# DCASE-REPO/DESED_task

Hardware: AMD Instinct MI355X
Metric: 10s-clips/sec CRNN mean-teacher train @batch48 (higher is better)
Workload: dtype f32 (fp32 storage and accumulation; the dense contractions of the wide layers run as split-bf16 MFMA, 3 bf16 products per fp32 product, fp32-level accuracy; everything else exact f32)

## Files before the change

desed_task_amd/_lib.py:

```python
import ctypes
import os
import re

_HERE = os.path.dirname(os.path.abspath(__file__))
_HEADER = os.path.join(os.path.dirname(_HERE), "include", "sed_hip.h")
LIB_PATH = os.path.join(_HERE, "libsed_hip.so")

_CTYPES = {"int": ctypes.c_int, "float": ctypes.c_float, "double": ctypes.c_double, "long long": ctypes.c_longlong,
           "unsigned": ctypes.c_uint, "unsigned int": ctypes.c_uint}

ERRORS = {-1: "bad argument", -2: "kernel launch failed", -3: "unsupported configuration"}


def parse_header(path=_HEADER):
    text = open(path).read()
    text = re.sub(r"/\*.*?\*/", "", text, flags=re.S)
    protos = {}
    for m in re.finditer(r"\b(?:int|long long)\s+(sed_\w+)\s*\(([^)]*)\)\s*;", text):
        args = []
        for a in m.group(2).split(","):
            a = a.strip()
            if "*" in a:
                args.append(ctypes.c_void_p)
            else:
                ty = re.sub(r"\bconst\b", "", a).strip()
                ty = ty.rsplit(None, 1)[0].strip()
                args.append(_CTYPES[ty])
        protos[m.group(1)] = args
    return protos


def header_constants(path=_HEADER):
    return {m.group(1): int(m.group(2)) for m in re.finditer(r"^#define\s+(SED_\w+)\s+(\d+)\b", open(path).read(), re.M)}


class _Lib:
    def __init__(self, path, is_emulator=False):
        self.path = path
        self.is_emulator = is_emulator
        import torch
        self._dll = ctypes.CDLL(path)
        self.protos = parse_header()
        for name, argtypes in self.protos.items():
            fn = getattr(self._dll, name)
            fn.argtypes = argtypes
            fn.restype = ctypes.c_longlong if name.endswith("_floats") else ctypes.c_int

    def value(self, name, *args):
        return getattr(self._dll, name)(*args)

    def call(self, name, *args):
        rc = getattr(self._dll, name)(*args)
        if rc != 0:
            raise RuntimeError("%s failed: %s (rc=%d)" % (name, ERRORS.get(rc, "?"), rc))


_lib = None


def get():
    global _lib
    if _lib is None:
        if not os.path.exists(LIB_PATH):
            raise RuntimeError(
                "desed_task_amd: %s is missing -- build it with `python -m desed_task_amd.build` "
                "(hipcc --offload-arch=gfx950).  There is no CPU fallback." % LIB_PATH)
        _lib = _Lib(LIB_PATH)
    return _lib


def use_library(path, is_emulator=True):
    global _lib
    _lib = _Lib(path, is_emulator=is_emulator) if path is not None else None
    return _lib


TUNING_KEYS = {"glu_grid_cap": 0, "glu_bwd128_split": 1, "convb_ck": 2, "convb_mp": 3, "block0_nocenter": 4, "glu_fwd128": 5, "wgrad_narrow": 6, "wgrad_cap": 7, "attn_valu": 8, "wgrad_wide": 9, "gru_lds_kb": 10, "mel_taps_mem": 11, "convb_tpw": 12, "mel_wave": 13, "gemm_ntn": 14, "linear_tiles": 15}


_tuning = {}


def set_tuning(key, value):
    get().call("sed_set_tuning", TUNING_KEYS[key], int(value))
    _tuning[key] = int(value)


def get_tuning(key):
    return _tuning.get(key, 0)


def check_tensor(t, name="tensor"):
    lib = get()
    if lib.is_emulator:
        if t.is_cuda:
            raise RuntimeError("%s: emulator build bound but tensor is on the GPU" % name)
    elif not t.is_cuda:
        raise RuntimeError("%s must live on the MI355X (cuda) device: there is no CPU path" % name)
    if not t.is_contiguous():
        raise RuntimeError("%s must be contiguous" % name)


def stream_ptr(t):
    if t.is_cuda:
        import torch
        return torch.cuda.current_stream(t.device).cuda_stream
    return 0
```

desed_task_amd/csrc/sed_common.h:

```cpp
#pragma once

#ifdef SED_EMU
#include "hip_emu.h"
#else
#include <hip/hip_runtime.h>
#define SED_DYN_SMEM(name) extern __shared__ __attribute__((aligned(16))) char name[]
#define SED_LAUNCH(kern, grid, block, smem, stream, ...) \
    hipLaunchKernelGGL(kern, grid, block, smem, stream, __VA_ARGS__)
typedef float f32x16 __attribute__((ext_vector_type(16)));
typedef float f32x4 __attribute__((ext_vector_type(4)));
typedef short s16x8 __attribute__((ext_vector_type(8)));
#endif

#include <stdint.h>

#define SED_API extern "C" __attribute__((visibility("default")))

#define SED_MAX_SMEM(kern, bytes) \
    (void)hipFuncSetAttribute((const void*)(kern), hipFuncAttributeMaxDynamicSharedMemorySize, (int)(bytes))

__global__ __launch_bounds__(256) static void sed_zero4_kernel(float* p0, int n0, float* p1, int n1, float* p2, int n2, float* p3, int n3) {
    const int i = blockIdx.x * 256 + threadIdx.x;
    if (i < n0) p0[i] = 0.f;
    if (i < n1) p1[i] = 0.f;
    if (i < n2) p2[i] = 0.f;
    if (i < n3) p3[i] = 0.f;
}
static inline void sed_zero4(hipStream_t s, float* p0, int n0, float* p1, int n1, float* p2, int n2, float* p3, int n3) {
    int n = n0 > n1 ? n0 : n1;
    n = n > n2 ? n : n2;
    n = n > n3 ? n : n3;
    if (n <= 0) return;
    SED_LAUNCH(sed_zero4_kernel, dim3((n + 255) / 256), dim3(256), 0, s, p0, n0, p1, n1, p2, n2, p3, n3);
}

#define SED_OK 0
#define SED_ERR_ARG (-1)
#define SED_ERR_LAUNCH (-2)
#define SED_ERR_UNSUPPORTED (-3)

enum { SED_TUNE_GLU_GRID_CAP = 0, SED_TUNE_GLU_BWD128_SPLIT = 1, SED_TUNE_CONVB_CK = 2, SED_TUNE_CONVB_MP = 3, SED_TUNE_B0_NOCENTER = 4, SED_TUNE_GLU_FWD128 = 5, SED_TUNE_WGRAD_NARROW = 6, SED_TUNE_WGRAD_CAP = 7,
       SED_TUNE_ATTN_VALU = 8, SED_TUNE_WGRAD_WIDE = 9, SED_TUNE_GRU_LDS_KB = 10, SED_TUNE_MEL_TAPS_MEM = 11, SED_TUNE_CONVB_TPW = 12, SED_TUNE_MEL_WAVE = 13, SED_TUNE_GEMM_NTN = 14, SED_TUNE_LINEAR_TILES = 15, SED_TUNE_COUNT = 16 };
extern int sed_tuning[SED_TUNE_COUNT];

static inline int sed_check_launch() {
    hipError_t e = hipGetLastError();
    return e == hipSuccess ? SED_OK : SED_ERR_LAUNCH;
}

__device__ __forceinline__ f32x16 mfma32(float a, float b, f32x16 c) {
#ifdef SED_EMU
    return emu_mfma_32x32x2(a, b, c);
#else
    return __builtin_amdgcn_mfma_f32_32x32x2f32(a, b, c, 0, 0, 0);
#endif
}
__device__ __forceinline__ int mfma32_row(int r, int lane) { return (r & 3) + 8 * (r >> 2) + 4 * (lane >> 5); }

__device__ __forceinline__ f32x4 mfma16(float a, float b, f32x4 c) {
#ifdef SED_EMU
    return emu_mfma_16x16x4(a, b, c);
#else
    return __builtin_amdgcn_mfma_f32_16x16x4f32(a, b, c, 0, 0, 0);
#endif
}

__device__ __forceinline__ f32x16 mfma32_bf16(s16x8 a, s16x8 b, f32x16 c) {
#ifdef SED_EMU
    return emu_mfma_32x32x16_bf16(a, b, c);
#else
    typedef __bf16 bf16x8_t __attribute__((ext_vector_type(8)));
    return __builtin_amdgcn_mfma_f32_32x32x16_bf16(__builtin_bit_cast(bf16x8_t, a), __builtin_bit_cast(bf16x8_t, b), c, 0, 0, 0);
#endif
}
__device__ __forceinline__ f32x4 mfma16_bf16(s16x8 a, s16x8 b, f32x4 c) {
#ifdef SED_EMU
    return emu_mfma_16x16x32_bf16(a, b, c);
#else
    typedef __bf16 bf16x8_t __attribute__((ext_vector_type(8)));
    return __builtin_amdgcn_mfma_f32_16x16x32_bf16(__builtin_bit_cast(bf16x8_t, a), __builtin_bit_cast(bf16x8_t, b), c, 0, 0, 0);
#endif
}
__device__ __forceinline__ unsigned short f32_to_bf16(float x) {
    unsigned u = __float_as_uint(x);
    u += 0x7FFFu + ((u >> 16) & 1u);
    return (unsigned short)(u >> 16);
}
__device__ __forceinline__ float bf16_to_f32(unsigned short h) { return __uint_as_float(((unsigned)h) << 16); }
__device__ __forceinline__ void bf16_split(float x, unsigned short& hi, unsigned short& lo) {
    hi = f32_to_bf16(x);
    lo = f32_to_bf16(x - bf16_to_f32(hi));
}

__device__ __forceinline__ float sed_sadd(float a, float b) {
#ifdef SED_EMU
    return a + b;
#else
    float r;
    asm("v_add_f32 %0, %1, %2" : "=v"(r) : "v"(a), "v"(b));
    return r;
#endif
}

__device__ __forceinline__ float sed_sfma(float a, float b, float c) {
#ifdef SED_EMU
    return fmaf(a, b, c);
#else
    float r;
    asm("v_fma_f32 %0, %1, %2, %3" : "=v"(r) : "v"(a), "v"(b), "v"(c));
    return r;
#endif
}

__device__ __forceinline__ void sed_sched_fence() {
#ifndef SED_EMU
    __builtin_amdgcn_sched_barrier(0);
#endif
}

__device__ __forceinline__ unsigned sed_alignbit(unsigned hi, unsigned lo, unsigned shift) {
#ifdef SED_EMU
    return (unsigned)(((((unsigned long long)hi) << 32) | lo) >> shift);
#else
    return __builtin_amdgcn_alignbit(hi, lo, shift);
#endif
}

template <class T_>
__device__ __forceinline__ void sed_pin(T_& x) {
#ifndef SED_EMU
    asm volatile("" : "+v"(x));
#else
    (void)x;
#endif
}
__device__ __forceinline__ void sed_opaque(int& x) {
#ifndef SED_EMU
    asm volatile("" : "+v"(x));
#else
    (void)x;
#endif
}

__device__ __forceinline__ int sed_wave_uniform(int x) {
#ifdef SED_EMU
    return x;
#else
    return __builtin_amdgcn_readfirstlane(x);
#endif
}

__device__ __forceinline__ void sed_wave_sync() {
#ifdef SED_EMU
    emu_wave_sync();
#else
    __builtin_amdgcn_fence(__ATOMIC_ACQ_REL, "wavefront");
    __builtin_amdgcn_wave_barrier();
#endif
}

__device__ __forceinline__ void bf16_split2(float a, float b, unsigned& hi, unsigned& lo) {
#ifdef SED_EMU
    unsigned short h0, l0, h1, l1;
    bf16_split(a, h0, l0);
    bf16_split(b, h1, l1);
    hi = (unsigned)h0 | ((unsigned)h1 << 16);
    lo = (unsigned)l0 | ((unsigned)l1 << 16);
#else
    typedef float f32x2_t __attribute__((ext_vector_type(2)));
    typedef __bf16 bf16x2_t __attribute__((ext_vector_type(2)));
    const f32x2_t v = {a, b};
    hi = __builtin_bit_cast(unsigned, __builtin_convertvector(v, bf16x2_t));
    const f32x2_t hf = {__uint_as_float(hi << 16), __uint_as_float(hi & 0xFFFF0000u)};
    lo = __builtin_bit_cast(unsigned, __builtin_convertvector(v - hf, bf16x2_t));
#endif
}
struct SedOneProduct {};
template <class... ONE>
constexpr int sed_np() { return sizeof...(ONE) ? 1 : 3; }
__device__ __forceinline__ unsigned bf16_round2(float a, float b) {
#ifdef SED_EMU
    return (unsigned)f32_to_bf16(a) | ((unsigned)f32_to_bf16(b) << 16);
#else
    typedef float f32x2_t __attribute__((ext_vector_type(2)));
    typedef __bf16 bf16x2_t __attribute__((ext_vector_type(2)));
    const f32x2_t v = {a, b};
    return __builtin_bit_cast(unsigned, __builtin_convertvector(v, bf16x2_t));
#endif
}

__device__ __forceinline__ f32x16 f32x16_zero() {
    f32x16 z;
#pragma unroll
    for (int i = 0; i < 16; ++i) z[i] = 0.f;
    return z;
}

__device__ __forceinline__ float sed_quad_xor1(float v) {
#ifdef SED_EMU
    return __shfl_xor(v, 1);
#else
    return __builtin_bit_cast(float, __builtin_amdgcn_update_dpp(0, __builtin_bit_cast(int, v), 0xB1, 0xF, 0xF, true));
#endif
}
__device__ __forceinline__ float sed_quad_xor2(float v) {
#ifdef SED_EMU
    return __shfl_xor(v, 2);
#else
    return __builtin_bit_cast(float, __builtin_amdgcn_update_dpp(0, __builtin_bit_cast(int, v), 0x4E, 0xF, 0xF, true));
#endif
}
__device__ __forceinline__ float sed_row_ror4(float v) {
#ifdef SED_EMU
    return __shfl_xor(v, 4);
#else
    return __builtin_bit_cast(float, __builtin_amdgcn_update_dpp(0, __builtin_bit_cast(int, v), 0x124, 0xF, 0xF, true));
#endif
}
__device__ __forceinline__ float sed_row_ror8(float v) {
#ifdef SED_EMU
    return __shfl_xor(v, 8);
#else
    return __builtin_bit_cast(float, __builtin_amdgcn_update_dpp(0, __builtin_bit_cast(int, v), 0x128, 0xF, 0xF, true));
#endif
}
__device__ __forceinline__ float sed_row16_max(float v) {
    v = fmaxf(v, sed_quad_xor1(v)); v = fmaxf(v, sed_quad_xor2(v));
    v = fmaxf(v, sed_row_ror4(v)); v = fmaxf(v, sed_row_ror8(v));
    return v;
}
__device__ __forceinline__ float sed_row16_sum(float v) {
    v += sed_quad_xor1(v); v += sed_quad_xor2(v);
    v += sed_row_ror4(v); v += sed_row_ror8(v);
    return v;
}
__device__ __forceinline__ float sed_half_mirror(float v) {
#ifdef SED_EMU
    return __shfl_xor(v, 7);
#else
    return __builtin_bit_cast(float, __builtin_amdgcn_update_dpp(0, __builtin_bit_cast(int, v), 0x141, 0xF, 0xF, true));
#endif
}
__device__ __forceinline__ float sed_quad_sum(float v) {
    v += sed_quad_xor1(v);
    v += sed_quad_xor2(v);
    return v;
}

__device__ __forceinline__ float wave_sum(float v) {
#pragma unroll
    for (int m = 32; m >= 1; m >>= 1) v += __shfl_xor(v, m);
    return v;
}
__device__ __forceinline__ float wave_min(float v) {
#pragma unroll
    for (int m = 32; m >= 1; m >>= 1) v = fminf(v, __shfl_xor(v, m));
    return v;
}
__device__ __forceinline__ float wave_max(float v) {
#pragma unroll
    for (int m = 32; m >= 1; m >>= 1) v = fmaxf(v, __shfl_xor(v, m));
    return v;
}

__device__ __forceinline__ uint32_t sed_mix32(uint32_t x) {
    x ^= x >> 16; x *= 0x85EBCA6Bu;
    x ^= x >> 13; x *= 0xC2B2AE35u;
    x ^= x >> 16;
    return x;
}
__device__ __forceinline__ uint32_t sed_hash(uint32_t idx, uint32_t seed) {
// ... 153 lines not shown
```

desed_task_amd/csrc/sed_conv.hip:

```cpp
#include "sed_common.h"

__global__ __launch_bounds__(256) void pack_weights_kernel(const float* __restrict__ W, float* __restrict__ Wf,
                                                           float* __restrict__ Wd, int COUT, int CIN) {
    const int i = blockIdx.x * 256 + threadIdx.x;
    if (i >= COUT * CIN * 9) return;
    const int b = i % 3, a = (i / 3) % 3, ci = (i / 9) % CIN, co = i / (9 * CIN);
    const float w = W[i];
    Wf[((a * 3 + b) * CIN + ci) * COUT + co] = w;
    if (Wd) Wd[(((2 - a) * 3 + (2 - b)) * COUT + co) * CIN + ci] = w;
}
SED_API int sed_conv_pack_weights(const float* W, float* Wf, float* Wd, int COUT, int CIN, void* stream) {
    const int n = COUT * CIN * 9;
    SED_LAUNCH(pack_weights_kernel, dim3((n + 255) / 256), dim3(256), 0, (hipStream_t)stream, W, Wf, Wd, COUT, CIN);
    return sed_check_launch();
}
struct PackJobs {
    const float* W[8];
    float* Wf[8];
    float* Wd[8];
    int cout[8], cin[8], start[9];
    int n;
};
__global__ __launch_bounds__(256) void pack_weights_multi_kernel(PackJobs jobs) {
    const int i = blockIdx.x * 256 + threadIdx.x;
// ... 463 lines not shown
            constexpr int NX = KT * (CIN / 4) / 256, ND = KT * (COUT / 4) / 256;
            float4 lx[NX], ldy[ND];
#pragma unroll
            for (int u = 0; u < NX; ++u) {
                const int idx = tid + 256 * u, r = idx / (CIN / 4), v = idx - r * (CIN / 4);
                const int p = p0 + r;
                lx[u] = make_float4(0.f, 0.f, 0.f, 0.f);
                if (p < npix) {
                    const int f = p % F, t = (p / F) % T, bb = p / (F * T);
                    const int t2 = t + da, f2 = f + db;
                    if (t2 >= 0 && t2 < T && f2 >= 0 && f2 < F)
                        lx[u] = *(const float4*)(x + (((size_t)bb * T + t2) * F + f2) * CIN + 4 * v);
                }
            }
#pragma unroll
            for (int u = 0; u < ND; ++u) {
                const int idx = tid + 256 * u, r = idx / (COUT / 4), v = idx - r * (COUT / 4);
                const int p = p0 + r;
                ldy[u] = make_float4(0.f, 0.f, 0.f, 0.f);
                if (p < npix) ldy[u] = *(const float4*)(dy + (size_t)p * COUT + 4 * v);
            }
#pragma unroll
            for (int u = 0; u < NX; ++u) {
                const int idx = tid + 256 * u, r = idx / (CIN / 4), v = idx - r * (CIN / 4);
                *(float4*)(xs + r * CIN + 4 * v) = lx[u];
            }
#pragma unroll
            for (int u = 0; u < ND; ++u) {
                const int idx = tid + 256 * u, r = idx / (COUT / 4), v = idx - r * (COUT / 4);
                *(float4*)(ds + r * COUT + 4 * v) = ldy[u];
            }
        }
        __syncthreads();
        constexpr int KS = KT / WK;
#pragma unroll 4
        for (int k = wk * KS; k < (wk + 1) * KS; k += 2) {
            float av[MT];
#pragma unroll
            for (int m = 0; m < MT; ++m) av[m] = (CIN >= 32 || lo < CIN) ? xs[(k + hi) * CIN + m * 32 + lo] : 0.f;
#pragma unroll
            for (int n = 0; n < NTW; ++n) {
                const int co = (wn * NTW + n) * 32 + lo;
                const float bv = (COUT >= 32 || lo < COUT) ? ds[(k + hi) * COUT + co] : 0.f;
#pragma unroll
                for (int m = 0; m < MT; ++m) acc[m][n] = mfma32(av[m], bv, acc[m][n]);
            }
        }
    }
    static_assert(WK == 1, "wide layers: every wave owns its output tiles");
    float* part = dWp + ((size_t)blockIdx.x * 9 + tap) * CIN * COUT;
#pragma unroll
    for (int m = 0; m < MT; ++m)
#pragma unroll
        for (int n = 0; n < NTW; ++n) {
            const int co = (wn * NTW + n) * 32 + lo;
#pragma unroll
            for (int r = 0; r < 16; ++r) {
                const int ci = m * 32 + mfma32_row(r, lane);
                if (ci < CIN && co < COUT) part[(size_t)ci * COUT + co] = acc[m][n][r];
            }
        }
}

template <int CIN, int COUT>
static int launch_wgrad(const float* x, const float* dy, float* dWp, int B, int T, int F, hipStream_t s) {
    using Cfg = WgCfg<CIN, COUT>;
    const int splits = wgrad_parts(CIN, COUT, B, T, F);
    SED_MAX_SMEM((conv_wgrad_kernel<CIN, COUT>), Cfg::SMEM);
    SED_LAUNCH((conv_wgrad_kernel<CIN, COUT>), dim3(splits, 9), dim3(256), Cfg::SMEM, s, x, dy, dWp, B, T, F);
    return sed_check_launch();
}

template <int CIN, int COUT, int NP = 3>
struct WgbCfg {
    static constexpr int PLANES = NP == 1 ? 1 : 2;
    static constexpr int KT = 64, RS = 64;
    static constexpr int MT = CIN / 32, NT = COUT / 32;
    static constexpr int WM = MT >= 4 ? 2 : 1, WN = 4 / WM;
    static constexpr int MTW = MT / WM, NTW = NT / WN;
    static constexpr int NBX = (KT / 4) * (CIN / 4) / 256, NBD = (KT / 4) * (COUT / 4) / 256;
    static constexpr int SMEM = PLANES * (CIN + COUT) * RS * 2;
    static_assert(NBX >= 1 && NBD >= 1 && MTW * WM == MT && NTW * WN == NT, "tile split");
};

template <bool LO = true>
__device__ __forceinline__ void wgb_store_row(float a, float b, float c, float d, unsigned short* __restrict__ hi_row,
                                              unsigned short* __restrict__ lo_row) {
    if constexpr (!LO) {
        *(uint2*)hi_row = make_uint2(bf16_round2(a, b), bf16_round2(c, d));
    } else {
    uint2 h, l;
    bf16_split2(a, b, h.x, l.x);
    bf16_split2(c, d, h.y, l.y);
    *(uint2*)hi_row = h;
    *(uint2*)lo_row = l;
    }
}
template <bool LO = true>
__device__ __forceinline__ void wgb_store_block(const float4 v0, const float4 v1, const float4 v2, const float4 v3,
                                                unsigned short* __restrict__ hi_plane, unsigned short* __restrict__ lo_plane,
                                                int cq, int pq, int RS) {
    const int r0 = 4 * cq, f0 = (r0 ^ cq) & 7;
    const int o0 = r0 * RS + 4 * (pq ^ (2 * f0)), o1 = (r0 + 1) * RS + 4 * (pq ^ (2 * (f0 ^ 1)));
    const int o2 = (r0 + 2) * RS + 4 * (pq ^ (2 * (f0 ^ 2))), o3 = (r0 + 3) * RS + 4 * (pq ^ (2 * (f0 ^ 3)));
    wgb_store_row<LO>(v0.x, v1.x, v2.x, v3.x, hi_plane + o0, lo_plane + o0);
    wgb_store_row<LO>(v0.y, v1.y, v2.y, v3.y, hi_plane + o1, lo_plane + o1);
    wgb_store_row<LO>(v0.z, v1.z, v2.z, v3.z, hi_plane + o2, lo_plane + o2);
    wgb_store_row<LO>(v0.w, v1.w, v2.w, v3.w, hi_plane + o3, lo_plane + o3);
}

template <int CIN, int COUT, class... ONE>
__global__ __launch_bounds__(256) void conv_wgrad_bf16_kernel(const float* __restrict__ x, const float* __restrict__ dy,
                                                              float* __restrict__ dWp, int B, int T, int F) {
    constexpr int NP = sed_np<ONE...>();
    using Cfg = WgbCfg<CIN, COUT, NP>;
    constexpr int KT = Cfg::KT, RS = Cfg::RS, WN = Cfg::WN, MTW = Cfg::MTW, NTW = Cfg::NTW, NBX = Cfg::NBX, NBD = Cfg::NBD;
    SED_DYN_SMEM(smem);
    unsigned short* xh = (unsigned short*)smem;
    unsigned short* xl = xh + (Cfg::PLANES - 1) * CIN * RS;
    unsigned short* dh = xl + CIN * RS;
    unsigned short* dl = dh + (Cfg::PLANES - 1) * COUT * RS;
    const int tid = threadIdx.x, lane = tid & 63, w = tid >> 6, lo = lane & 31, hi = lane >> 5;
    const int wn = w % WN, wm = w / WN;
    const int tap = blockIdx.y, da = tap / 3 - 1, db = tap % 3 - 1;
    const int npix = B * T * F;
    const int ntiles = (npix + KT - 1) / KT;
    const int fsh = 31 - __builtin_clz(F);

    f32x16 acc[MTW][NTW];
#pragma unroll
    for (int m = 0; m < MTW; ++m)
#pragma unroll
        for (int n = 0; n < NTW; ++n) acc[m][n] = f32x16_zero();

    float4 rx[NBX * 4], rd[NBD * 4];
    unsigned okx = 0, okd = 0;
    static_assert(NBX * 4 <= 32 && NBD * 4 <= 32, "validity masks");
    auto load_tile = [&](int tile) {
        const int p0 = tile * KT;
        okx = 0; okd = 0;
#pragma unroll
        for (int u = 0; u < NBX; ++u) {
            const int blk = tid + 256 * u, cq = (blk >> 1) % (CIN / 4), pq = (blk & 1) + 2 * ((blk >> 1) / (CIN / 4));
#pragma unroll
            for (int j = 0; j < 4; ++j) {
                const int p = p0 + 4 * pq + j, pc = p < npix ? p : 0;
                const int f = pc & (F - 1), tt = pc >> fsh, t = tt % T, bb = tt / T;
                const int t2 = t + da, f2 = f + db;
                const bool ok = p < npix && t2 >= 0 && t2 < T && f2 >= 0 && f2 < F;
                okx |= (ok ? 1u : 0u) << (4 * u + j);
                const int t2c = t2 < 0 ? 0 : (t2 >= T ? T - 1 : t2), f2c = f2 < 0 ? 0 : (f2 >= F ? F - 1 : f2);
                rx[4 * u + j] = *(const float4*)(x + (((size_t)bb * T + t2c) * F + f2c) * CIN + 4 * cq);
            }
        }
#pragma unroll
        for (int u = 0; u < NBD; ++u) {
            const int blk = tid + 256 * u, cq = (blk >> 1) % (COUT / 4), pq = (blk & 1) + 2 * ((blk >> 1) / (COUT / 4));
#pragma unroll
            for (int j = 0; j < 4; ++j) {
                const int p = p0 + 4 * pq + j;
                okd |= (p < npix ? 1u : 0u) << (4 * u + j);
                rd[4 * u + j] = *(const float4*)(dy + (size_t)(p < npix ? p : 0) * COUT + 4 * cq);
            }
        }
    };
    auto store_tile = [&]() {
#pragma unroll
        for (int i = 0; i < NBX * 4; ++i) if (!((okx >> i) & 1u)) rx[i] = make_float4(0.f, 0.f, 0.f, 0.f);
#pragma unroll
        for (int i = 0; i < NBD * 4; ++i) if (!((okd >> i) & 1u)) rd[i] = make_float4(0.f, 0.f, 0.f, 0.f);
#pragma unroll
        for (int u = 0; u < NBX; ++u) {
            const int blk = tid + 256 * u;
            wgb_store_block<NP != 1>(rx[4 * u], rx[4 * u + 1], rx[4 * u + 2], rx[4 * u + 3], xh, xl, (blk >> 1) % (CIN / 4),
                            (blk & 1) + 2 * ((blk >> 1) / (CIN / 4)), RS);
        }
#pragma unroll
        for (int u = 0; u < NBD; ++u) {
            const int blk = tid + 256 * u;
            wgb_store_block<NP != 1>(rd[4 * u], rd[4 * u + 1], rd[4 * u + 2], rd[4 * u + 3], dh, dl, (blk >> 1) % (COUT / 4),
                            (blk & 1) + 2 * ((blk >> 1) / (COUT / 4)), RS);
        }
    };

    int tile = blockIdx.x;
    if (tile < ntiles) load_tile(tile);
    for (; tile < ntiles; tile += gridDim.x) {
        __syncthreads();
        store_tile();
        __syncthreads();
        if (tile + (int)gridDim.x < ntiles) load_tile(tile + gridDim.x);
#pragma unroll
// ... 784 lines not shown
```

desed_task_amd/csrc/sed_gemm_bf16.hip:

```cpp
#include "sed_common.h"

namespace {

constexpr int GB_BM = 128, GB_BK = 32, GB_RS = 40;

__device__ __forceinline__ void split4(const float4 v, uint2& h, uint2& l) {
    bf16_split2(v.x, v.y, h.x, l.x);
    bf16_split2(v.z, v.w, h.y, l.y);
}
__device__ __forceinline__ uint2 round4(const float4 v) { return make_uint2(bf16_round2(v.x, v.y), bf16_round2(v.z, v.w)); }

template <int ROWS, bool KC>
struct OperandTile {
    static constexpr int NV = ROWS * GB_BK / 4 / 256;
    float4 r[NV];
    static __device__ __forceinline__ int kc_row(int i) {
        const int grp = i >> 4;
        return ((grp >> 2) << 3) + (grp & 3) + ((i >> 1) & 4);
    }
    __device__ __forceinline__ void load(const float* __restrict__ base, int ld, int row0, int nrows, int k0, int kend, int tid) {
#pragma unroll
        for (int u = 0; u < NV; ++u) {
            r[u] = make_float4(0.f, 0.f, 0.f, 0.f);
            if (KC) {
// ... 48 lines not shown
    }
};

template <int TA, int TB, int NTN, class... ONE>
__global__ __launch_bounds__(256, 3) void gemm_bf16x3_kernel(const float* __restrict__ A, const float* __restrict__ Bm,
                                                          const float* __restrict__ bias, float* __restrict__ Cm, int M, int N, int K,
                                                          int lda, int ldb, int ldc, int k_per_slice, int atomic,
                                                          const float* __restrict__ A1, const float* __restrict__ B1,
                                                          const float* __restrict__ bias1, float* __restrict__ C1, int nbatch,
                                                          const float* __restrict__ Bsw, int ksw, int act, float* __restrict__ part,
                                                          int walk_nt) {
    constexpr int NP = sed_np<ONE...>();
    constexpr int BM = GB_BM, BN = 32 * NTN, BK = GB_BK, RS = GB_RS;
    constexpr int PLANES = NP == 1 ? 1 : 2;
    __shared__ __attribute__((aligned(16))) unsigned short As[PLANES * BM * RS];
    __shared__ __attribute__((aligned(16))) unsigned short Bs[PLANES * BN * RS];
    const int tid = threadIdx.x, lane = tid & 63, w = tid >> 6, lo = lane & 31, hi = lane >> 5;
    int tile_m = blockIdx.y, tile_n = blockIdx.x;
    if (walk_nt > 0) {
        const int ml = blockIdx.x >> 3;
        tile_m = (blockIdx.x & 7) + 8 * (ml / walk_nt);
        tile_n = ml % walk_nt;
        if (tile_m * BM >= M) return;
    }
    const int m0 = tile_m * BM, n0 = tile_n * BN;
    const int zb = nbatch == 2 ? (blockIdx.z & 1) : 0, zs = nbatch == 2 ? (blockIdx.z >> 1) : blockIdx.z;
    if (zb) { A = A1; Bm = B1; bias = bias1; Cm = C1; }
    if (part) { Cm = part + (size_t)blockIdx.z * M * N; ldc = N; }
    const int kbeg = zs * k_per_slice, kend = min(K, kbeg + k_per_slice);
    f32x16 acc[NTN];
#pragma unroll
    for (int i = 0; i < NTN; ++i) acc[i] = f32x16_zero();
    OperandTile<BM, TA == 0> ta;
    OperandTile<BN, TB == 1> tb;

    if (kbeg < kend) { ta.load(A, lda, m0, M, kbeg, kend, tid); tb.load((Bsw && kbeg >= ksw) ? Bsw : Bm, ldb, n0, N, kbeg, kend, tid); }
    for (int k0 = kbeg; k0 < kend; k0 += BK) {
        __syncthreads();
        ta.template store<NP != 1>(As, As + BM * RS, tid);
        tb.template store<NP != 1>(Bs, Bs + BN * RS, tid);
        __syncthreads();
        if (k0 + BK < kend) { ta.load(A, lda, m0, M, k0 + BK, kend, tid); tb.load((Bsw && k0 + BK >= ksw) ? Bsw : Bm, ldb, n0, N, k0 + BK, kend, tid); }
        const unsigned short* ap = As + (32 * w + lo) * RS + 8 * hi;
#pragma unroll
        for (int ks = 0; ks < BK / 16; ++ks) {
            const s16x8 a_hi = *(const s16x8*)(ap + 16 * ks);
            if constexpr (NP == 1) {
#pragma unroll
                for (int nt = 0; nt < NTN; ++nt)
                    acc[nt] = mfma32_bf16(a_hi, *(const s16x8*)(Bs + (nt * 32 + lo) * RS + 16 * ks + 8 * hi), acc[nt]);
            } else {
            const s16x8 a_lo = *(const s16x8*)(ap + BM * RS + 16 * ks);
#pragma unroll
            for (int nt = 0; nt < NTN; ++nt) {
                const unsigned short* bp = Bs + (nt * 32 + lo) * RS + 16 * ks + 8 * hi;
                const s16x8 b_hi = *(const s16x8*)bp;
                const s16x8 b_lo = *(const s16x8*)(bp + BN * RS);
                acc[nt] = mfma32_bf16(a_lo, b_hi, acc[nt]);
                acc[nt] = mfma32_bf16(a_hi, b_lo, acc[nt]);
                acc[nt] = mfma32_bf16(a_hi, b_hi, acc[nt]);
            }
            }
        }
    }
#pragma unroll
    for (int nt = 0; nt < NTN; ++nt) {
        const int gn = n0 + nt * 32 + lo;
        if (gn < N) {
            const float bv = (bias != nullptr && zs == 0) ? bias[gn] : 0.f;
#pragma unroll
            for (int r = 0; r < 16; ++r) {
                const int gm = m0 + 32 * w + mfma32_row(r, lane);
                if (gm < M) {
                    float* dst = Cm + (size_t)gm * ldc + gn;
                    float v = acc[nt][r] + bv;
                    if (act == 1) v = 0.5f * v * (1.0f + erff(v * 0.70710678118654752f));
                    if (atomic) atomicAdd(dst, v); else *dst = v;
                }
            }
        }
    }
}

}

SED_API int sed_gemm(const float* A, const float* Bm, const float* bias, float* Cm, int M, int N, int K, int lda, int ldb,
                        int ldc, int transA, int transB, int split_k, int accumulate, void* stream);
SED_API int sed_gemm_pair(const float* A0, const float* A1, const float* B0, const float* B1, const float* bias0,
                             const float* bias1, float* C0, float* C1, int M, int N, int K, int lda, int ldb, int ldc, int transA,
                             int transB, int split_k, int accumulate, void* stream);

static int gemmb_dispatch(const float* A, const float* Bm, const float* bias, float* Cm, const float* A1, const float* B1,
                          const float* bias1, float* C1, int nbatch, int M, int N, int K, int lda, int ldb, int ldc, int transA,
                          int transB, int split_k, int accumulate, hipStream_t s, const float* Bsw = nullptr, int ksw = 0, int act = 0,
                          float* part = nullptr, bool act_linear = false, bool single = false) {
    if (M <= 0 || N <= 0 || K <= 0) return SED_OK;
    bool ok = ((uintptr_t)A % 16 == 0) && ((uintptr_t)Bm % 16 == 0) && lda % 4 == 0 && ldb % 4 == 0 &&
              ((transA ? M : K) % 4 == 0) && ((transB ? K : N) % 4 == 0) && !(transA && transB);
    if (nbatch == 2) ok = ok && ((uintptr_t)A1 % 16 == 0) && ((uintptr_t)B1 % 16 == 0);
    if (!ok && (Bsw || act || part)) return SED_ERR_UNSUPPORTED;
    if (!ok) {
        if (nbatch == 2) return sed_gemm_pair(A, A1, Bm, B1, bias, bias1, Cm, C1, M, N, K, lda, ldb, ldc, transA, transB, split_k, accumulate, s);
        return sed_gemm(A, Bm, bias, Cm, M, N, K, lda, ldb, ldc, transA, transB, split_k, accumulate, s);
    }
    if (split_k < 1) split_k = 1;
    int kps = ((K + split_k - 1) / split_k + 31) / 32 * 32;
    split_k = (K + kps - 1) / kps;
    const int atomic = (!part && (split_k > 1 || accumulate)) ? 1 : 0;
    int ntn = N > 64 ? 4 : 2;
    if (ntn == 4 && ((N + 127) / 128) * ((M + 127) / 128) * split_k * nbatch < 400) ntn = 2;
    if (ntn == 4 && !transA && transB && N % 96 == 0) {
        const long long rows = (M + 127) / 128, z = (long long)split_k * nbatch, slots = 768;
        const long long t4 = rows * ((N + 127) / 128) * z, t3 = rows * (N / 96) * z;
        if (sed_tuning[SED_TUNE_GEMM_NTN] == 3) ntn = 3;
        else if (t4 > slots) {
            const double e4 = (double)t4 / (double)(((t4 + slots - 1) / slots) * slots), e3 = (double)t3 / (double)(((t3 + slots - 1) / slots) * slots);
            if (e3 > e4 + 0.1) ntn = 3;
        }
    }
    dim3 grid((N + 32 * ntn - 1) / (32 * ntn), (M + 127) / 128, split_k * nbatch);
    int walk_nt = 0;
    if (act_linear && split_k * nbatch == 1 && grid.y >= 16) {
        walk_nt = (int)grid.x;
        grid = dim3(grid.x * ((grid.y + 7) / 8) * 8, 1, 1);
    }
#define GEMMB_CASE(ta, tb, nn) \
    if (single && transA == ta && transB == tb && ntn == nn) { SED_LAUNCH((gemm_bf16x3_kernel<ta, tb, nn, SedOneProduct>), grid, dim3(256), 0, s, A, Bm, bias, Cm, M, N, K, lda, ldb, ldc, kps, atomic, A1, B1, bias1, C1, nbatch, Bsw, ksw, act, part, walk_nt); return sed_check_launch(); }
    GEMMB_CASE(0, 0, 2) GEMMB_CASE(0, 0, 4) GEMMB_CASE(0, 1, 2) GEMMB_CASE(0, 1, 3) GEMMB_CASE(0, 1, 4) GEMMB_CASE(1, 0, 2) GEMMB_CASE(1, 0, 4)
#undef GEMMB_CASE
#define GEMMB_CASE(ta, tb, nn) \
    if (transA == ta && transB == tb && ntn == nn) { SED_LAUNCH((gemm_bf16x3_kernel<ta, tb, nn>), grid, dim3(256), 0, s, A, Bm, bias, Cm, M, N, K, lda, ldb, ldc, kps, atomic, A1, B1, bias1, C1, nbatch, Bsw, ksw, act, part, walk_nt); return sed_check_launch(); }
    GEMMB_CASE(0, 0, 2) GEMMB_CASE(0, 0, 4) GEMMB_CASE(0, 1, 2) GEMMB_CASE(0, 1, 3) GEMMB_CASE(0, 1, 4) GEMMB_CASE(1, 0, 2) GEMMB_CASE(1, 0, 4)
#undef GEMMB_CASE
    return SED_ERR_UNSUPPORTED;
}

SED_API int sed_gemm_bf16x3(const float* A, const float* Bm, const float* bias, float* Cm, int M, int N, int K, int lda, int ldb,
                               int ldc, int transA, int transB, int split_k, int accumulate, void* stream) {
    return gemmb_dispatch(A, Bm, bias, Cm, nullptr, nullptr, nullptr, nullptr, 1, M, N, K, lda, ldb, ldc, transA, transB, split_k,
                          accumulate, (hipStream_t)stream);
}
SED_API int sed_gemm_pair_bf16x3(const float* A0, const float* A1, const float* B0, const float* B1, const float* bias0,
                                    const float* bias1, float* C0, float* C1, int M, int N, int K, int lda, int ldb, int ldc,
                                    int transA, int transB, int split_k, int accumulate, void* stream) {
    return gemmb_dispatch(A0, B0, bias0, C0, A1, B1, bias1, C1, 2, M, N, K, lda, ldb, ldc, transA, transB, split_k, accumulate,
                          (hipStream_t)stream);
}

__global__ __launch_bounds__(256) void splitk_reduce_kernel(const float* __restrict__ part, float* __restrict__ C0, float* __restrict__ C1,
                                                            int nslices, int M, int N, int ldc) {
    const int MN4 = M * N / 4, i = blockIdx.x * 256 + threadIdx.x, zb = blockIdx.y, nb = gridDim.y;
    if (i >= MN4) return;
    const float4* src = (const float4*)part + (size_t)zb * MN4 + i;
    float4 acc = make_float4(0.f, 0.f, 0.f, 0.f);
#pragma unroll 4
    for (int z = 0; z < nslices; ++z) {
        const float4 v = src[(size_t)nb * z * MN4];
        acc.x += v.x; acc.y += v.y; acc.z += v.z; acc.w += v.w;
    }
    const int e = 4 * i, m = e / N, n = e - m * N;
    *(float4*)((zb ? C1 : C0) + (size_t)m * ldc + n) = acc;
}
static inline int splitk_slices(int K, int split_k) {
    if (split_k < 1) split_k = 1;
    const int kps = ((K + split_k - 1) / split_k + 31) / 32 * 32;
    return (K + kps - 1) / kps;
}
SED_API long long sed_gemm_splitk_scratch_floats(int M, int N, int K, int split_k) {
    return 2LL * splitk_slices(K, split_k) * M * N;
}
SED_API int sed_gemm_pair_splitk_bf16x3(const float* A0, const float* A1, const float* B0, const float* B1, float* C0, float* C1,
                                           int M, int N, int K, int lda, int ldb, int ldc, int transA, int transB, int split_k,
                                           float* scratch, void* stream) {
    if (M <= 0 || N <= 0) return SED_OK;
    if (!scratch || N % 4 != 0 || ldc % 4 != 0 || K <= 0) return SED_ERR_ARG;
    if ((((uintptr_t)C0 | (uintptr_t)C1) & 15) != 0) return SED_ERR_UNSUPPORTED;
    hipStream_t s = (hipStream_t)stream;
    const int rc = gemmb_dispatch(A0, B0, nullptr, C0, A1, B1, nullptr, C1, 2, M, N, K, lda, ldb, ldc, transA, transB, split_k, 0, s,
                                  nullptr, 0, 0, scratch);
    if (rc != SED_OK) return rc;
    SED_LAUNCH(splitk_reduce_kernel, dim3((M * N / 4 + 255) / 256, 2), dim3(256), 0, s, (const float*)scratch, C0, C1,
               splitk_slices(K, split_k), M, N, ldc);
    return sed_check_launch();
}

SED_API int sed_gemm_splitk_bf16x3(const float* A, const float* Bm, float* Cm, int M, int N, int K, int lda, int ldb, int ldc,
                                   int transA, int transB, int split_k, float* scratch, void* stream) {
    if (M <= 0 || N <= 0) return SED_OK;
    if (!scratch || N % 4 != 0 || ldc % 4 != 0 || K <= 0) return SED_ERR_ARG;
    if (((uintptr_t)Cm & 15) != 0) return SED_ERR_UNSUPPORTED;
    hipStream_t s = (hipStream_t)stream;
// ... 728 lines not shown
```

desed_task_amd/csrc/sed_selftest.hip:

```cpp
#include "sed_common.h"

int sed_tuning[SED_TUNE_COUNT] = {0};
SED_API int sed_set_tuning(int key, int value) {
    if (key < 0 || key >= SED_TUNE_COUNT) return SED_ERR_ARG;
    sed_tuning[key] = value;
    return SED_OK;
}

__global__ __launch_bounds__(64) void selftest_mfma32_kernel(const float* A, const float* Bm, float* C, int K) {
    const int lane = threadIdx.x;
    f32x16 acc = f32x16_zero();
    for (int k = 0; k < K; k += 2) {
        const float a = A[(lane & 31) * K + k + (lane >> 5)];
        const float b = Bm[(k + (lane >> 5)) * 32 + (lane & 31)];
        acc = mfma32(a, b, acc);
    }
#pragma unroll
    for (int r = 0; r < 16; ++r) C[mfma32_row(r, lane) * 32 + (lane & 31)] = acc[r];
}
__global__ __launch_bounds__(64) void selftest_mfma16_kernel(const float* A, const float* Bm, float* C, int K) {
    const int lane = threadIdx.x;
    f32x4 acc = {0.f, 0.f, 0.f, 0.f};
    for (int k = 0; k < K; k += 4) {
        const float a = A[(lane & 15) * K + k + (lane >> 4)];
        const float b = Bm[(k + (lane >> 4)) * 16 + (lane & 15)];
        acc = mfma16(a, b, acc);
    }
#pragma unroll
    for (int r = 0; r < 4; ++r) C[((lane >> 4) * 4 + r) * 16 + (lane & 15)] = acc[r];
}
__global__ __launch_bounds__(64) void selftest_mfma32_bf16_kernel(const float* A, const float* Bm, float* C, int K) {
    const int lane = threadIdx.x;
    f32x16 acc = f32x16_zero();
    for (int k = 0; k < K; k += 16) {
        s16x8 a, b;
#pragma unroll
        for (int e = 0; e < 8; ++e) {
            const int kk = k + 8 * (lane >> 5) + e;
            a[e] = (short)f32_to_bf16(A[(lane & 31) * K + kk]);
            b[e] = (short)f32_to_bf16(Bm[kk * 32 + (lane & 31)]);
        }
        acc = mfma32_bf16(a, b, acc);
    }
#pragma unroll
    for (int r = 0; r < 16; ++r) C[mfma32_row(r, lane) * 32 + (lane & 31)] = acc[r];
}
__global__ __launch_bounds__(64) void selftest_mfma16_bf16_kernel(const float* A, const float* Bm, float* C, int K) {
    const int lane = threadIdx.x;
    f32x4 acc = {0.f, 0.f, 0.f, 0.f};
    for (int k = 0; k < K; k += 32) {
        s16x8 a, b;
#pragma unroll
        for (int e = 0; e < 8; ++e) {
            const int kk = k + 8 * (lane >> 4) + e;
            a[e] = (short)f32_to_bf16(A[(lane & 15) * K + kk]);
            b[e] = (short)f32_to_bf16(Bm[kk * 16 + (lane & 15)]);
        }
        acc = mfma16_bf16(a, b, acc);
    }
#pragma unroll
    for (int r = 0; r < 4; ++r) C[((lane >> 4) * 4 + r) * 16 + (lane & 15)] = acc[r];
}
SED_API int sed_selftest_mfma(const float* A, const float* Bm, float* C, int K, int shape, void* stream) {
    if (shape == 32) SED_LAUNCH(selftest_mfma32_kernel, dim3(1), dim3(64), 0, (hipStream_t)stream, A, Bm, C, K);
    else if (shape == 3216) SED_LAUNCH(selftest_mfma32_bf16_kernel, dim3(1), dim3(64), 0, (hipStream_t)stream, A, Bm, C, K);
    else if (shape == 1632) SED_LAUNCH(selftest_mfma16_bf16_kernel, dim3(1), dim3(64), 0, (hipStream_t)stream, A, Bm, C, K);
    else if (shape == 16) SED_LAUNCH(selftest_mfma16_kernel, dim3(1), dim3(64), 0, (hipStream_t)stream, A, Bm, C, K);
    else return SED_ERR_ARG;
    return sed_check_launch();
}
```

Before: 16310.

## Add k-major GEMM kernel for transposed-A weight-gradient split-K path

Adds a dedicated GEMM kernel for the transA, non-transB, partial-output case. It loads K-major float4 columns of A and B, splits them into bf16 hi/lo planes in swizzled LDS, and accumulates with 3-product bf16 MFMA. Loads for the next K tile are issued while the current tile is being multiplied, and work items are spread across the 8 XCDs. The kernel is on by default through a new tuning key, and the shared store helpers move into the common header. The added costs are more registers per thread and a new code path whose strided loads could be slower than the existing kernel for some shapes.

```diff
diff --git a/desed_task_amd/_lib.py b/desed_task_amd/_lib.py
--- a/desed_task_amd/_lib.py
+++ b/desed_task_amd/_lib.py
@@ -75,7 +75,8 @@
     return _lib
 
 
-TUNING_KEYS = {"glu_grid_cap": 0, "glu_bwd128_split": 1, "convb_ck": 2, "convb_mp": 3, "block0_nocenter": 4, "glu_fwd128": 5, "wgrad_narrow": 6, "wgrad_cap": 7, "attn_valu": 8, "wgrad_wide": 9, "gru_lds_kb": 10, "mel_taps_mem": 11, "convb_tpw": 12, "mel_wave": 13, "gemm_ntn": 14, "linear_tiles": 15}
+TUNING_KEYS = {"glu_grid_cap": 0, "glu_bwd128_split": 1, "convb_ck": 2, "convb_mp": 3, "block0_nocenter": 4, "glu_fwd128": 5, "wgrad_narrow": 6, "wgrad_cap": 7, "attn_valu": 8, "wgrad_wide": 9, "gru_lds_kb": 10, "mel_taps_mem": 11, "convb_tpw": 12, "mel_wave": 13, "gemm_ntn": 14, "linear_tiles": 15,
+               "gemm_kmajor": 16}
 
 
 _tuning = {}
diff --git a/desed_task_amd/csrc/sed_common.h b/desed_task_amd/csrc/sed_common.h
--- a/desed_task_amd/csrc/sed_common.h
+++ b/desed_task_amd/csrc/sed_common.h
@@ -40,7 +40,7 @@
 #define SED_ERR_UNSUPPORTED (-3)
 
 enum { SED_TUNE_GLU_GRID_CAP = 0, SED_TUNE_GLU_BWD128_SPLIT = 1, SED_TUNE_CONVB_CK = 2, SED_TUNE_CONVB_MP = 3, SED_TUNE_B0_NOCENTER = 4, SED_TUNE_GLU_FWD128 = 5, SED_TUNE_WGRAD_NARROW = 6, SED_TUNE_WGRAD_CAP = 7,
-       SED_TUNE_ATTN_VALU = 8, SED_TUNE_WGRAD_WIDE = 9, SED_TUNE_GRU_LDS_KB = 10, SED_TUNE_MEL_TAPS_MEM = 11, SED_TUNE_CONVB_TPW = 12, SED_TUNE_MEL_WAVE = 13, SED_TUNE_GEMM_NTN = 14, SED_TUNE_LINEAR_TILES = 15, SED_TUNE_COUNT = 16 };
+       SED_TUNE_ATTN_VALU = 8, SED_TUNE_WGRAD_WIDE = 9, SED_TUNE_GRU_LDS_KB = 10, SED_TUNE_MEL_TAPS_MEM = 11, SED_TUNE_CONVB_TPW = 12, SED_TUNE_MEL_WAVE = 13, SED_TUNE_GEMM_NTN = 14, SED_TUNE_LINEAR_TILES = 15, SED_TUNE_GEMM_KMAJOR = 16, SED_TUNE_COUNT = 17 };
 extern int sed_tuning[SED_TUNE_COUNT];
 
 static inline int sed_check_launch() {
@@ -187,6 +187,32 @@
     const f32x2_t v = {a, b};
     return __builtin_bit_cast(unsigned, __builtin_convertvector(v, bf16x2_t));
 #endif
+}
+
+template <bool LO = true>
+__device__ __forceinline__ void wgb_store_row(float a, float b, float c, float d, unsigned short* __restrict__ hi_row,
+                                              unsigned short* __restrict__ lo_row) {
+    if constexpr (!LO) {
+        *(uint2*)hi_row = make_uint2(bf16_round2(a, b), bf16_round2(c, d));
+    } else {
+    uint2 h, l;
+    bf16_split2(a, b, h.x, l.x);
+    bf16_split2(c, d, h.y, l.y);
+    *(uint2*)hi_row = h;
+    *(uint2*)lo_row = l;
+    }
+}
+template <bool LO = true>
+__device__ __forceinline__ void wgb_store_block(const float4 v0, const float4 v1, const float4 v2, const float4 v3,
+                                                unsigned short* __restrict__ hi_plane, unsigned short* __restrict__ lo_plane,
+                                                int cq, int pq, int RS) {
+    const int r0 = 4 * cq, f0 = (r0 ^ cq) & 7;
+    const int o0 = r0 * RS + 4 * (pq ^ (2 * f0)), o1 = (r0 + 1) * RS + 4 * (pq ^ (2 * (f0 ^ 1)));
+    const int o2 = (r0 + 2) * RS + 4 * (pq ^ (2 * (f0 ^ 2))), o3 = (r0 + 3) * RS + 4 * (pq ^ (2 * (f0 ^ 3)));
+    wgb_store_row<LO>(v0.x, v1.x, v2.x, v3.x, hi_plane + o0, lo_plane + o0);
+    wgb_store_row<LO>(v0.y, v1.y, v2.y, v3.y, hi_plane + o1, lo_plane + o1);
+    wgb_store_row<LO>(v0.z, v1.z, v2.z, v3.z, hi_plane + o2, lo_plane + o2);
+    wgb_store_row<LO>(v0.w, v1.w, v2.w, v3.w, hi_plane + o3, lo_plane + o3);
 }
 
 __device__ __forceinline__ f32x16 f32x16_zero() {
diff --git a/desed_task_amd/csrc/sed_conv.hip b/desed_task_amd/csrc/sed_conv.hip
--- a/desed_task_amd/csrc/sed_conv.hip
+++ b/desed_task_amd/csrc/sed_conv.hip
@@ -569,32 +569,6 @@
     static constexpr int SMEM = PLANES * (CIN + COUT) * RS * 2;
     static_assert(NBX >= 1 && NBD >= 1 && MTW * WM == MT && NTW * WN == NT, "tile split");
 };
-
-template <bool LO = true>
-__device__ __forceinline__ void wgb_store_row(float a, float b, float c, float d, unsigned short* __restrict__ hi_row,
-                                              unsigned short* __restrict__ lo_row) {
-    if constexpr (!LO) {
-        *(uint2*)hi_row = make_uint2(bf16_round2(a, b), bf16_round2(c, d));
-    } else {
-    uint2 h, l;
-    bf16_split2(a, b, h.x, l.x);
-    bf16_split2(c, d, h.y, l.y);
-    *(uint2*)hi_row = h;
-    *(uint2*)lo_row = l;
-    }
-}
-template <bool LO = true>
-__device__ __forceinline__ void wgb_store_block(const float4 v0, const float4 v1, const float4 v2, const float4 v3,
-                                                unsigned short* __restrict__ hi_plane, unsigned short* __restrict__ lo_plane,
-                                                int cq, int pq, int RS) {
-    const int r0 = 4 * cq, f0 = (r0 ^ cq) & 7;
-    const int o0 = r0 * RS + 4 * (pq ^ (2 * f0)), o1 = (r0 + 1) * RS + 4 * (pq ^ (2 * (f0 ^ 1)));
-    const int o2 = (r0 + 2) * RS + 4 * (pq ^ (2 * (f0 ^ 2))), o3 = (r0 + 3) * RS + 4 * (pq ^ (2 * (f0 ^ 3)));
-    wgb_store_row<LO>(v0.x, v1.x, v2.x, v3.x, hi_plane + o0, lo_plane + o0);
-    wgb_store_row<LO>(v0.y, v1.y, v2.y, v3.y, hi_plane + o1, lo_plane + o1);
-    wgb_store_row<LO>(v0.z, v1.z, v2.z, v3.z, hi_plane + o2, lo_plane + o2);
-    wgb_store_row<LO>(v0.w, v1.w, v2.w, v3.w, hi_plane + o3, lo_plane + o3);
-}
 
 template <int CIN, int COUT, class... ONE>
 __global__ __launch_bounds__(256) void conv_wgrad_bf16_kernel(const float* __restrict__ x, const float* __restrict__ dy,
diff --git a/desed_task_amd/csrc/sed_gemm_bf16.hip b/desed_task_amd/csrc/sed_gemm_bf16.hip
--- a/desed_task_amd/csrc/sed_gemm_bf16.hip
+++ b/desed_task_amd/csrc/sed_gemm_bf16.hip
@@ -154,6 +154,154 @@
     }
 }
 
+template <int NTN, class... ONE>
+__global__ __launch_bounds__(256, NTN == 2 ? 3 : 2) void gemm_kmajor_kernel(const float* __restrict__ A, const float* __restrict__ Bm, int M, int N,
+                                                                           int K, int lda, int ldb, int k_per_slice,
+                                                                           const float* __restrict__ A1, const float* __restrict__ B1,
+                                                                           int nbatch, float* __restrict__ part, int tiles_n, int tiles_m) {
+    constexpr int NP = sed_np<ONE...>(), PLANES = NP == 1 ? 1 : 2;
+    constexpr int BM = GB_BM, BN = 32 * NTN, KT = 64, RS = 64;
+    constexpr int NBA = (KT / 4) * (BM / 4) / 256, NBB = (KT / 4) * (BN / 4) / 256;
+    static_assert(NBA * 256 == (KT / 4) * (BM / 4) && NBB * 256 == (KT / 4) * (BN / 4) && NBB >= 1, "tile split");
+    SED_DYN_SMEM(smem);
+    unsigned short* ah = (unsigned short*)smem;
+    unsigned short* al = ah + (PLANES - 1) * BM * RS;
+    unsigned short* bh = al + BM * RS;
+    unsigned short* bl = bh + (PLANES - 1) * BN * RS;
+    const int tid = threadIdx.x, lane = tid & 63, w = tid >> 6, lo = lane & 31, hi = lane >> 5;
+    const int nwg = gridDim.x, xcd = blockIdx.x & 7, per = nwg >> 3, rem = nwg & 7;
+    const int item = xcd * per + min(xcd, rem) + (int)(blockIdx.x >> 3);
+    const int tile_n = item % tiles_n, rest = item / tiles_n, tile_m = rest % tiles_m, z = rest / tiles_m;
+    const int m0 = tile_m * BM, n0 = tile_n * BN;
+    const int zb = nbatch == 2 ? (z & 1) : 0, zs = nbatch == 2 ? (z >> 1) : z;
+    if (zb) { A = A1; Bm = B1; }
+    const int kbeg = zs * k_per_slice, kend = min(K, kbeg + k_per_slice);
+
+    f32x16 acc[NTN];
+#pragma unroll
+    for (int i = 0; i < NTN; ++i) acc[i] = f32x16_zero();
+
+    float4 ra[NBA * 4], rb[NBB * 4];
+    unsigned oka = 0, okb = 0;
+    auto load_tile = [&](int k0) {
+        oka = 0; okb = 0;
+#pragma unroll
+        for (int u = 0; u < NBA; ++u) {
+            const int blk = tid + 256 * u, cq = (blk >> 1) % (BM / 4), pq = (blk & 1) + 2 * ((blk >> 1) / (BM / 4));
+            const int gm = m0 + 4 * cq;
+            const float* col = A + (gm < M ? gm : 0);
+#pragma unroll
+            for (int j = 0; j < 4; ++j) {
+                const int gk = k0 + 4 * pq + j;
+                oka |= ((gk < kend && gm < M) ? 1u : 0u) << (4 * u + j);
+                ra[4 * u + j] = *(const float4*)(col + (size_t)(gk < kend ? gk : kend - 1) * lda);
+            }
+        }
+#pragma unroll
+        for (int u = 0; u < NBB; ++u) {
+            const int blk = tid + 256 * u, cq = (blk >> 1) % (BN / 4), pq = (blk & 1) + 2 * ((blk >> 1) / (BN / 4));
+            const int gn = n0 + 4 * cq;
+            const float* col = Bm + (gn < N ? gn : 0);
+#pragma unroll
+            for (int j = 0; j < 4; ++j) {
+                const int gk = k0 + 4 * pq + j;
+                okb |= ((gk < kend && gn < N) ? 1u : 0u) << (4 * u + j);
+                rb[4 * u + j] = *(const float4*)(col + (size_t)(gk < kend ? gk : kend - 1) * ldb);
+            }
+        }
+    };
+    auto store_tile = [&]() {
+#pragma unroll
+        for (int i = 0; i < NBA * 4; ++i) if (!((oka >> i) & 1u)) ra[i] = make_float4(0.f, 0.f, 0.f, 0.f);
+#pragma unroll
+        for (int i = 0; i < NBB * 4; ++i) if (!((okb >> i) & 1u)) rb[i] = make_float4(0.f, 0.f, 0.f, 0.f);
+#pragma unroll
+        for (int u = 0; u < NBA; ++u) {
+            const int blk = tid + 256 * u;
+            wgb_store_block<NP != 1>(ra[4 * u], ra[4 * u + 1], ra[4 * u + 2], ra[4 * u + 3], ah, al, (blk >> 1) % (BM / 4),
+                                     (blk & 1) + 2 * ((blk >> 1) / (BM / 4)), RS);
+        }
+#pragma unroll
+        for (int u = 0; u < NBB; ++u) {
+            const int blk = tid + 256 * u;
+            wgb_store_block<NP != 1>(rb[4 * u], rb[4 * u + 1], rb[4 * u + 2], rb[4 * u + 3], bh, bl, (blk >> 1) % (BN / 4),
+                                     (blk & 1) + 2 * ((blk >> 1) / (BN / 4)), RS);
+        }
+    };
+
+    const int arow = 32 * w + lo, af = (arow ^ (arow >> 2)) & 7;
+    auto mma_tile = [&](int k0) {
+#pragma unroll
+        for (int ks = 0; ks < KT / 16; ++ks) {
+            if (k0 + 16 * ks >= kend) break;
+            const int oct = 2 * ks + hi;
+            const int aoff = arow * RS + 8 * (oct ^ af);
+            const s16x8 a_hi = *(const s16x8*)(ah + aoff);
+            if constexpr (NP == 1) {
+#pragma unroll
+                for (int nt = 0; nt < NTN; ++nt) {
+                    const int row = nt * 32 + lo;
+                    acc[nt] = mfma32_bf16(a_hi, *(const s16x8*)(bh + row * RS + 8 * (oct ^ ((row ^ (row >> 2)) & 7))), acc[nt]);
+                }
+            } else {
+            const s16x8 a_lo = *(const s16x8*)(al + aoff);
+#pragma unroll
+            for (int nt = 0; nt < NTN; ++nt) {
+                const int row = nt * 32 + lo;
+                const int off = row * RS + 8 * (oct ^ ((row ^ (row >> 2)) & 7));
+                const s16x8 b_hi = *(const s16x8*)(bh + off);
+                const s16x8 b_lo = *(const s16x8*)(bl + off);
+                acc[nt] = mfma32_bf16(a_lo, b_hi, acc[nt]);
+                acc[nt] = mfma32_bf16(a_hi, b_lo, acc[nt]);
+                acc[nt] = mfma32_bf16(a_hi, b_hi, acc[nt]);
+            }
+            }
+        }
+    };
+
+    load_tile(kbeg);
+    int k0 = kbeg;
+    for (; k0 + KT < kend; k0 += KT) {
+        __syncthreads();
+        store_tile();
+        __syncthreads();
+        load_tile(k0 + KT);
+        mma_tile(k0);
+    }
+    __syncthreads();
+    store_tile();
+    __syncthreads();
+    mma_tile(k0);
+    float* dst = part + (size_t)z * M * N;
+#pragma unroll
+    for (int nt = 0; nt < NTN; ++nt) {
+        const int gn = n0 + nt * 32 + lo;
+        if (gn < N) {
+#pragma unroll
+            for (int r = 0; r < 16; ++r) {
+                const int gm = m0 + 32 * w + mfma32_row(r, lane);
+                if (gm < M) dst[(size_t)gm * N + gn] = acc[nt][r];
+            }
+        }
+    }
+}
+
+template <int NTN, bool SINGLE>
+static int launch_kmajor(const float* A, const float* Bm, const float* A1, const float* B1, int nbatch, int M, int N, int K, int lda,
+                         int ldb, int kps, int slices, float* part, hipStream_t s) {
+    constexpr int SMEM = (SINGLE ? 1 : 2) * (GB_BM + 32 * NTN) * 64 * 2;
+    const int tiles_n = (N + 32 * NTN - 1) / (32 * NTN), tiles_m = (M + GB_BM - 1) / GB_BM;
+    const dim3 grid(tiles_n * tiles_m * slices * nbatch);
+    if constexpr (SINGLE) {
+        SED_MAX_SMEM((gemm_kmajor_kernel<NTN, SedOneProduct>), SMEM);
+        SED_LAUNCH((gemm_kmajor_kernel<NTN, SedOneProduct>), grid, dim3(256), SMEM, s, A, Bm, M, N, K, lda, ldb, kps, A1, B1, nbatch, part, tiles_n, tiles_m);
+    } else {
+        SED_MAX_SMEM((gemm_kmajor_kernel<NTN>), SMEM);
+        SED_LAUNCH((gemm_kmajor_kernel<NTN>), grid, dim3(256), SMEM, s, A, Bm, M, N, K, lda, ldb, kps, A1, B1, nbatch, part, tiles_n, tiles_m);
+    }
+    return sed_check_launch();
+}
+
 }
 
 SED_API int sed_gemm(const float* A, const float* Bm, const float* bias, float* Cm, int M, int N, int K, int lda, int ldb,
@@ -179,6 +327,14 @@
     int kps = ((K + split_k - 1) / split_k + 31) / 32 * 32;
     split_k = (K + kps - 1) / kps;
     const int atomic = (!part && (split_k > 1 || accumulate)) ? 1 : 0;
+    if (transA && !transB && part && !Bsw && !act && sed_tuning[SED_TUNE_GEMM_KMAJOR] != 0) {
+        const long long wg2 = (long long)((N + 63) / 64) * ((M + 127) / 128) * split_k * nbatch;
+        if (wg2 <= 768 || N <= 64)
+            return single ? launch_kmajor<2, true>(A, Bm, A1, B1, nbatch, M, N, K, lda, ldb, kps, split_k, part, s)
+                          : launch_kmajor<2, false>(A, Bm, A1, B1, nbatch, M, N, K, lda, ldb, kps, split_k, part, s);
+        return single ? launch_kmajor<4, true>(A, Bm, A1, B1, nbatch, M, N, K, lda, ldb, kps, split_k, part, s)
+                      : launch_kmajor<4, false>(A, Bm, A1, B1, nbatch, M, N, K, lda, ldb, kps, split_k, part, s);
+    }
     int ntn = N > 64 ? 4 : 2;
     if (ntn == 4 && ((N + 127) / 128) * ((M + 127) / 128) * split_k * nbatch < 400) ntn = 2;
     if (ntn == 4 && !transA && transB && N % 96 == 0) {
diff --git a/desed_task_amd/csrc/sed_selftest.hip b/desed_task_amd/csrc/sed_selftest.hip
--- a/desed_task_amd/csrc/sed_selftest.hip
+++ b/desed_task_amd/csrc/sed_selftest.hip
@@ -1,6 +1,6 @@
 #include "sed_common.h"
 
-int sed_tuning[SED_TUNE_COUNT] = {0};
+int sed_tuning[SED_TUNE_COUNT] = {0, 0, 0, 0, 0, 0, 0, 0, 0, 0, 0, 0, 0, 0, 0, 0,  1};
 SED_API int sed_set_tuning(int key, int value) {
     if (key < 0 || key >= SED_TUNE_COUNT) return SED_ERR_ARG;
     sed_tuning[key] = value;
```

Result: no change. 16360 (median of 6 runs) (+0.3%).
